# rpng/open_vins

Measured on AMD Instinct MI355X. Metric: MSCKF features/sec per EKF update (30-clone state), higher is better.
Workload: dtype f64; 1 GPU; BASELINE.json configs[2]: 2-camera radtan rig, 30-clone window, 2000 MSCKF features/update, N=248, D=208, online cam extrinsic+intrinsic calib + IMU intrinsics in the state, FEJ; features_total=2000, features_this_rank=2000, clones=30, cameras=2, state_dim=248, measurements_total=100362, parallelism=single GPU

## Files before the change

open_vins_amd/csrc/api_context.inc:

```
using namespace ovg;

static thread_local std::string g_err = "";
static int set_err(int code, const std::string &msg) {
  g_err = msg;
  return code;
}

#define HIPCHK(expr)                                                                                         \
  do {                                                                                                       \
    hipError_t _e = (expr);                                                                                  \
    if (_e != hipSuccess) {                                                                                  \
      return set_err(OVGPU_ERR_HIP, std::string(#expr) + " -> " + hipGetErrorString(_e) + " (" __FILE__ ":" + \
                                        std::to_string(__LINE__) + ")");                                     \
    }                                                                                                        \
  } while (0)

namespace {

template <class T>
struct PinBuf {
  T *p = nullptr;
  size_t cap = 0;
  hipError_t reserve(size_t n) {
    if (n <= cap) return hipSuccess;
// ... 234 lines not shown
  int tree_G = 0;
  bool tree_pipelined = true;
  int compress_gram = 1;
  DevBuf<double> gram_part, gram_G, gram_rho, Yaug2, Lw;
  double prior_pivot_tol = 1e-13;
  int last_route = OVGPU_COMPRESS_GRAM;
  bool whiten = true;
  bool gram_is_whitened = false;
  bool prior_on_side = false;
  int feat_variant = 0;
  int feat_nt_max = 0;
  bool featy_ok = false;
  int featy_skip = 0;
  int featy_grid = 0;
  size_t featy_lds = 0;
  DevBuf<double> fs_tq;
  DevBuf<int32_t> fs_inst;
  DevBuf<double> featyb_ws;
  int featy_big = 0;
  bool no_feat_kernel = false;
  bool raw_enable = true;
  bool gram_read_ahead = true;
  bool featy_chains = true;
  int raw_work_const = 12;
  bool raw_veto = false;
  bool raw_one_region = false;
  bool raw_cols_ok = false;
  bool raw_tables_ok = false;
  int raw_j0 = 0;
  int raw_ncls = 0, raw_ntc[RAW_MAXCLS + 1] = {0}, raw_ld[RAW_MAXCLS + 1] = {0}, raw_rcol[RAW_MAXCLS + 1] = {0};
  int64_t raw_base[RAW_MAXCLS + 1] = {0}, raw_rows[RAW_MAXCLS + 1] = {0};
  std::vector<uint8_t> h_cls_of_clone;
  DevBuf<uint8_t> cls_of_clone;
  DevBuf<int32_t> raw_featbase, raw_dst, raw_runs;
  DevBuf<double> Hraw;
  DevBuf<gram::GramRegionWG> gram_wg;
  int gram_wg_n = 0, gram_wg_tiles = 0;
  gram::GramRegionSum raw_rs;
  bool last_stack_raw = false;
  DevView<int32_t> feat_counter;
  DevBuf<int32_t> fs_minfo, fs_meas_feat, fs_pos;
  DevBuf<int32_t> fs_slots;
  std::vector<int32_t> h_order;
  std::vector<uint16_t> h_cc;
  DevBuf<double> fs_rows, fs_V, fs_z, fs_w;
  void *comm = nullptr;
// ... 344 lines not shown
```

open_vins_amd/csrc/api_debug.inc:

```
int ovgpu_debug_option(ovgpu_ctx *c, const char *name, int64_t value, int64_t *old_value) {
  if (!c || !name) return set_err(OVGPU_ERR_INVALID, "null argument");
  const std::string n(name);
  if (n == "chol_follow_spin_limit") {
    if (old_value) *old_value = c->chol_spin_limit;
    if (value >= 0) c->chol_spin_limit = (int)std::min<int64_t>(value, 1 << 30);
  } else if (n == "slam_chunked_fail_chunk") {
    if (old_value) *old_value = c->chunk_fail_inject;
    c->chunk_fail_inject = value >= 0 ? (int)std::min<int64_t>(value, 1 << 20) : -1;
  } else if (n == "slam_chunked_fallbacks") {
    if (old_value) *old_value = c->chunk_fallbacks;
    if (value >= 0) c->chunk_fallbacks = value;
  } else if (n == "delayed_init_fused") {
    if (old_value) *old_value = c->init_fused_on ? 1 : 0;
    if (value >= 0) c->init_fused_on = value != 0;
  } else if (n == "delayed_init_fused_steps") {
    if (old_value) *old_value = c->init_fused_steps;
    if (value >= 0) c->init_fused_steps = value;
  } else if (n == "delayed_init_chain_steps") {
    if (old_value) *old_value = c->init_chain_steps;
    if (value >= 0) c->init_chain_steps = value;
  } else if (n == "gram_interleaved") {
    if (old_value) *old_value = c->gram_il ? 1 : 0;
    if (value >= 0) c->gram_il = value != 0;
  } else if (n == "layout_fpw") {
// ... 34 lines not shown
    if (value >= 0) c->featy_big = (int)value;
  } else if (n == "upload_kernel") {
    if (old_value) *old_value = c->up_kernel;
    if (value >= 0) c->up_kernel = value != 0;
  } else if (n == "layout_every_update") {
    if (old_value) *old_value = c->layout_every_update;
    if (value >= 0) c->layout_every_update = value != 0;
  } else if (n == "tri_waves") {
    if (old_value) *old_value = c->tri_waves;
    if (value >= 0 && value <= 16) c->tri_waves = (int)value;
  } else if (n == "featy_skip") {
#ifdef OVG_FEAT_ABLATE
    if (old_value) *old_value = c->featy_skip;
    if (value >= 0) c->featy_skip = (int)value;
#else
    return set_err(OVGPU_ERR_INVALID, "featy_skip: ablation switches exist in a developer build only (-DOVG_FEAT_ABLATE)");
#endif
  } else if (n == "gram_read_ahead") {
    if (old_value) *old_value = c->gram_read_ahead ? 1 : 0;
    if (value >= 0) c->gram_read_ahead = value != 0;
  } else if (n == "featy_chains") {
    if (old_value) *old_value = c->featy_chains ? 1 : 0;
    if (value >= 0) c->featy_chains = value != 0;
  } else if (n == "raw_work_const") {
    if (old_value) *old_value = c->raw_work_const;
    if (value >= 0) c->raw_work_const = (int)value;
  } else if (n == "last_stack_raw") {
    if (old_value) *old_value = c->last_stack_raw ? 1 : 0;
  } else if (n == "raw_gram_tile_rows") {
    int64_t t = 0;
    if (c->raw_tables_ok)
      for (int k = 0; k <= RAW_NEG; k++) t += c->raw_rows[k] * (int64_t)(c->raw_ntc[k] * (c->raw_ntc[k] + 1) / 2);
    if (old_value) *old_value = t;
  } else if (n == "stack_is_f32") {
    if (old_value) *old_value = c->stack_is_f32 ? 1 : 0;
  } else if (n == "last_feature_kernel") {
    if (old_value) *old_value = c->last_feat_kernel;
  } else if (n == "last_gram_kernel") {
    if (old_value) *old_value = c->last_gram_kernel;
  } else if (n == "last_factor_kernel") {
    if (old_value) *old_value = c->last_factor_kernel;
  } else if (n == "last_unwhiten_kernel") {
    if (old_value) *old_value = c->last_unwhiten_kernel;
  } else if (n == "chol_wide") {
    if (old_value) *old_value = c->chol_wide ? 1 : 0;
    if (value >= 0) c->chol_wide = value != 0;
// ... 8 lines not shown
    if (old_value) *old_value = c->tsqr_last_leaf;
  } else if (n == "tsqr_last_tree") {
    if (old_value) *old_value = c->tsqr_last_tree;
  } else if (n == "tsqr_last_qh") {
    if (old_value) *old_value = c->tsqr_last_qh;
  } else if (n == "sys_lds_limit") {
    if (old_value) *old_value = c->lds_limit;
  } else if (n == "sys_m_lds_max") {
    if (old_value) *old_value = c->m_lds_max;
  } else if (n == "sys_rows_global") {
    if (old_value) *old_value = c->sys_rows_global ? 1 : 0;
  } else if (n == "sys_row_stride") {
    if (old_value) *old_value = c->row_stride;
  } else if (n == "sys_lds_bytes") {
    if (old_value) *old_value = (int64_t)c->sys_lds_bytes;
  } else if (n == "chol_timeouts") {
    if (old_value) *old_value = c->chol_timeouts;
  } else {
    return set_err(OVGPU_ERR_INVALID, "unknown debug option");
  }
  return OVGPU_OK;
}

int ovgpu_debug_cycles(ovgpu_ctx *c, int enable, long long *out512) {
  if (!c) return set_err(OVGPU_ERR_INVALID, "null ctx");
  HIPCHK(hipSetDevice(c->device));
  HIPCHK(upload_sync(c, c->stream));
  if (out512 && c->dbg_cycles.p) HIPCHK(hipMemcpy(out512, c->dbg_cycles.p, 512 * sizeof(long long), hipMemcpyDeviceToHost));
  if (enable) {
    HIPCHK(c->dbg_cycles.reserve(512));
    HIPCHK(hipMemset(c->dbg_cycles.p, 0, 512 * sizeof(long long)));
  } else if (!out512) {
    c->dbg_cycles.release();
  }
  return OVGPU_OK;
}

#ifdef OVG_GRAM_PROF
extern "C" int ovgpu_debug_gram_phases(ovgpu_ctx *c, long long *out, int workgroups, int *launched) {
  if (!c || !out || !launched || workgroups < 0 || workgroups > 1024) return set_err(OVGPU_ERR_INVALID, "bad argument");
  *launched = c->gram_wg_n;
  HIPCHK(hipSetDevice(c->device));
  HIPCHK(upload_sync(c, c->stream));
  HIPCHK(hipMemcpyFromSymbol(out, HIP_SYMBOL(gram::gram_prof_buf), sizeof(long long) * 32 * workgroups));
  return OVGPU_OK;
}
#endif

__global__ void k_clock_probe(long long *out, int iters) {
  const long long c0 = clock64(), w0 = wall_clock64();
  unsigned x = threadIdx.x + 1;
  for (int i = 0; i < iters; i++) x = x * 1664525u + 1013904223u;
  const long long c1 = clock64(), w1 = wall_clock64();
  if (threadIdx.x == 0) out[0] = c1 - c0, out[1] = w1 - w0, out[2] = (long long)x;
}
__global__ void __launch_bounds__(256) k_clock_probe_load(long long *out, int iters) {
  typedef double d4 __attribute__((ext_vector_type(4)));
  d4 a0 = {0, 0, 0, 0}, a1 = a0, a2 = a0, a3 = a0;
  const double x = 1.0 + 1e-9 * threadIdx.x, y = 1.0 - 1e-9 * threadIdx.x;
// ... 133 lines not shown
```

open_vins_amd/csrc/api_pipeline.inc:

```
static int enqueue_triangulate(ovgpu_ctx *c, const double *seed_pA = nullptr, const int32_t *seed_anchor = nullptr) {
  const Batch b = batch_of(c);
  if (b.F == 0) return OVGPU_OK;
  TriParams p;
  p.seed_pA = seed_pA, p.seed_anchor = seed_anchor, p.anchor_pre = c->anchor_pre.p;
  p.F = b.F, p.C = c->C, p.K = c->K;
  p.meas_offsets = b.meas_offsets, p.meas_cc = b.meas_cc, p.uvn = b.uvn, p.tab_cc = c->tab_cc.p;
  p.p_FinA = b.pA, p.p_FinG = b.pG, p.anchor_meas = c->anchor.p, p.status = b.status;
  p.opt = c->dopt;
  const size_t lds = (size_t)c->K * c->C * 12 * sizeof(double);
  int wpb = c->tri_waves;
  if (wpb == 0) {
    wpb = 4;
    const int room = c->num_cu - 6;
    for (int w = 4; w <= 8 && room > 0; w *= 2) {
      const int blocks = (b.F + w - 1) / w;
      if (blocks <= room) {
        if (4 * blocks >= 3 * room) wpb = w;
        break;
      }
    }
  }
  hipLaunchKernelGGL(k_triangulate, dim3((b.F + wpb - 1) / wpb), dim3(64 * wpb), lds, c->stream, p);
  HIPCHK(hipGetLastError());
  return OVGPU_OK;
}

extern "C++" {
template <int NW, int TPW, int OCC, bool F32, int CB, bool CH = false>
static int launch_featy(ovgpu_ctx *c, const SysParams &p, const double *sr, const int32_t *sm, const double *sV, const double *stq, const int32_t *sin, const int32_t *ssl) {
  static bool attr = false;
  auto kern = feat::k_feat_y<NW, TPW, OCC, F32, CB, CH>;
  if (!attr) {
    (void)hipFuncSetAttribute((const void *)kern, hipFuncAttributeMaxDynamicSharedMemorySize, c->lds_limit);
    attr = true;
  }
  const int nt = c->feat_nt_max, nta = c->feat_nta_max;
  if (nta * (nta + 1) / 2 > NW * TPW) return set_err(OVGPU_ERR_INVALID, "internal: the fused kernel's shape does not hold this batch's longest track");
  const size_t lds = feat::featy_lds_layout(nt, nta, NW, CB).total;
  if (lds > (size_t)c->lds_limit) return set_err(OVGPU_ERR_CAPACITY, "k_feat_y: track too long for its LDS block");
  const int per_cu = std::max(1, std::min(std::max(1, 4 * OCC / NW), (int)((size_t)c->lds_limit / lds)));
  const int grid = std::max(1, std::min(batch_of(c).F, c->num_cu * per_cu));
  hipLaunchKernelGGL(kern, dim3(grid), dim3(64 * NW), lds, c->stream, p, nt, nta, sr, sm, sV, stq, sin, ssl, (const int32_t *)c->raw_runs.p);
  return OVGPU_OK;
}
}

static int enqueue_system(ovgpu_ctx *c, int f_one = -1, int init_rep = 0, bool whiten = false) {
  const Batch b = batch_of(c);
  if (b.F == 0) return OVGPU_OK;
  SysParams p;
  p.F = b.F, p.C = c->C, p.K = c->K, p.D = c->D, p.LD = c->LD, p.N = c->N;
  p.meas_offsets = b.meas_offsets, p.meas_cc = b.meas_cc, p.uv = b.uv;
  p.tab_clone = c->tab_clone.p, p.tab_cam = c->tab_cam.p, p.intr = c->intr.p, p.fisheye = c->fisheye.p;
  p.clone_col = c->clone_col.p, p.calib_col = c->calib_col.p, p.intr_col = c->intr_col.p;
  p.col_cov = c->col_cov.p, p.col_kind = c->col_kind.p, p.col_var = c->col_var.p, p.col_sub = c->col_sub.p;
  p.P = c->P.p, p.p_FinG = b.pG, p.p_FinA = b.pA, p.anchor_meas = c->anchor.p;
  p.status = b.status, p.chi2 = b.chi2, p.chi2_thresh = b.chi2_thr;
  p.chi2_table = c->chi2_table.p, p.chi2_table_len = c->chi2_table_len;
  p.row_off = b.row_off, p.Hbig = c->Hbig.p, p.ws = c->gate_ws.p, p.ws_stride = c->gate_ws_stride;
  p.Hbig32 = nullptr, p.LDF = 0;
  c->stack_is_f32 = false;
  p.m_lds_max = c->m_lds_max, p.m_max = std::max(b.m_max, 1), p.row_stride = c->row_stride;
  p.opt = c->dopt;
  p.dbg = c->dbg_cycles.p ? c->dbg_cycles.p : qr_dbg_buffer();
// ... 51 lines not shown
        p.raw.on = 1, p.raw.ncls = c->raw_ncls, p.raw.H = c->Hraw.p, p.raw.dst = c->raw_dst.p, p.raw.j0 = c->raw_j0;
        for (int k = 0; k <= RAW_NEG; k++) p.raw.base[k] = c->raw_base[k], p.raw.ld[k] = c->raw_ld[k], p.raw.rcol[k] = c->raw_rcol[k];
        c->last_stack_raw = true;
      }
      if (c->inst_cb != cb || c->inst_D != c->D) {
        const int rci = enqueue_instance_lists(c, cb);
        if (rci != OVGPU_OK) return rci;
      }
      hipLaunchKernelGGL(feat::k_feat_vt, dim3((b.F + 3) / 4), dim3(256), (size_t)4 * (14 * p.m_max + 64) * sizeof(double), c->stream, p, st, c->fs_tq.p);
      if (c->prior_on_side) {
        HIPCHK(hipStreamWaitEvent(c->stream, c->ev_join, 0));
        c->prior_on_side = false;
      }
      const double *stq = c->fs_tq.p;
      const int32_t *sin = c->fs_inst.p, *ssl = c->fs_slots.p;
      if (big) {
        static bool attr_b = false;
        if (!attr_b) {
          (void)hipFuncSetAttribute((const void *)feat::k_feat_y_big<8, 17>, hipFuncAttributeMaxDynamicSharedMemorySize, c->lds_limit);
          (void)hipFuncSetAttribute((const void *)feat::k_feat_y_big<8, 17, true>, hipFuncAttributeMaxDynamicSharedMemorySize, c->lds_limit);
          (void)hipFuncSetAttribute((const void *)feat::k_feat_y_big<8, 5>, hipFuncAttributeMaxDynamicSharedMemorySize, c->lds_limit);
          attr_b = true;
        }
        const int nt = c->feat_nt_max, gridb = std::max(1, std::min(b.F, c->num_cu));
        const size_t ldsb = feat::featyb_lds_layout(nt, 8).total;
        if (ldsb > (size_t)c->lds_limit || nt > 29) return set_err(OVGPU_ERR_CAPACITY, "k_feat_y_big: track too long for its LDS block");
        HIPCHK(c->featyb_ws.reserve((size_t)gridb * feat::featyb_ws_doubles(nt)));
        if (c->featy_big == 2) hipLaunchKernelGGL((feat::k_feat_y_big<8, 5>), dim3(gridb), dim3(512), ldsb, c->stream, p, nt, sr, sm, sV, stq, sin, ssl, c->featyb_ws.p);
        else if (p.Hbig32) hipLaunchKernelGGL((feat::k_feat_y_big<8, 17, true>), dim3(gridb), dim3(512), ldsb, c->stream, p, nt, sr, sm, sV, stq, sin, ssl, c->featyb_ws.p);
        else hipLaunchKernelGGL((feat::k_feat_y_big<8, 17>), dim3(gridb), dim3(512), ldsb, c->stream, p, nt, sr, sm, sV, stq, sin, ssl, c->featyb_ws.p);
      } else {
        int rcl;
        if (c->feat_variant == 1 && p.Hbig32) rcl = launch_featy<4, 9, 2, true, 64>(c, p, sr, sm, sV, stq, sin, ssl);
        else if (c->feat_variant == 1) rcl = c->featy_chains ? launch_featy<4, 9, 2, false, 64, true>(c, p, sr, sm, sV, stq, sin, ssl) : launch_featy<4, 9, 2, false, 64>(c, p, sr, sm, sV, stq, sin, ssl);
        else if (p.Hbig32) rcl = launch_featy<8, 17, 1, true, 64>(c, p, sr, sm, sV, stq, sin, ssl);
        else rcl = c->featy_chains ? launch_featy<8, 17, 1, false, 64, true>(c, p, sr, sm, sV, stq, sin, ssl) : launch_featy<8, 17, 1, false, 64>(c, p, sr, sm, sV, stq, sin, ssl);
        if (rcl != OVGPU_OK) return rcl;
      }
      HIPCHK(hipGetLastError());
      return OVGPU_OK;
    }
    return set_err(OVGPU_ERR_INVALID, "internal: the MSCKF fast path was selected for a batch the fused kernel does not hold");
  }
  if (p.Lw && c->prior_on_side) {
    HIPCHK(hipStreamWaitEvent(c->stream, c->ev_join, 0));
    c->prior_on_side = false;
  }
// ... 982 lines not shown
```

open_vins_amd/csrc/api_state.inc:

```

const char *ovgpu_last_error(void) { return g_err.c_str(); }

void ovgpu_default_options(ovgpu_options *o) {
  if (!o) return;
  std::memset(o, 0, sizeof(*o));
  o->chi2_multipler = 5.0, o->sigma_pix = 1.0;
  o->triangulate_1d = 0, o->refine_features = 1, o->max_runs = 5;
  o->init_lamda = 1e-3, o->max_lamda = 1e10, o->min_dx = 1e-6, o->min_dcost = 1e-6, o->lam_mult = 10;
  o->min_dist = 0.10, o->max_dist = 60, o->max_baseline = 40, o->max_cond_number = 10000;
  o->do_fej = 1, o->do_calib_camera_pose = 1, o->do_calib_camera_intrinsics = 1;
  o->feat_rep_msckf = OVGPU_REP_GLOBAL_3D;
}

double ovgpu_chi2_quantile_95(int dof) { return chi2_quantile_95(dof); }
int ovgpu_abi_version(void) { return OVGPU_ABI_VERSION; }

int ovgpu_create(const ovgpu_options *opts, int device, ovgpu_ctx **out) {
  if (!opts || !out) return set_err(OVGPU_ERR_INVALID, "null argument");
  *out = nullptr;
  int ndev = 0;
  hipError_t e = hipGetDeviceCount(&ndev);
  if (e != hipSuccess || ndev <= 0)
    return set_err(OVGPU_ERR_NO_DEVICE, std::string("no HIP device (") + hipGetErrorString(e) + "): this library has no CPU fallback");
  if (device < 0 || device >= ndev) return set_err(OVGPU_ERR_INVALID, "device index out of range");
// ... 475 lines not shown
  c->inst_cb = lists ? cb : 0, c->inst_D = c->D;
  return OVGPU_OK;
}
static int enqueue_instance_lists(ovgpu_ctx *c, int cb) { return enqueue_batch_layout(c, false, cb); }
static int enqueue_batch_tables(ovgpu_ctx *c, bool anchors) { return enqueue_batch_layout(c, anchors, c->featy_ok ? featy_block_cols(c, featy_stack_f32(c, -1)) : feat::FY_CB); }

static int feature_rows(bool slam_rows, int m, int proj) { return slam_rows ? std::max(2 * m - proj, 0) : (m >= 2 ? 2 * m - 3 : 0); }
static void row_offsets_of(const ovgpu_ctx *c, const Batch &b, bool slam_rows, int64_t *out) {
  const int udof = lm_uniform_dof(c);
  out[0] = 0;
  for (int f = 0; f < b.F; f++) {
    int proj = udof == 1 ? 2 : 0;
    if (udof == 0 && (int)b.h_feat_lm.size() == b.F) proj = 3 - lm_dof(c->h_lm_rep[b.h_feat_lm[f]]);
    out[f + 1] = out[f] + feature_rows(slam_rows, b.h_offsets[f + 1] - b.h_offsets[f], proj);
  }
}
static void track_order(const int32_t *offsets, int F, int m_max, int32_t *order) {
  std::vector<int32_t> start(m_max + 2, 0);
  for (int f = 0; f < F; f++) start[m_max - (offsets[f + 1] - offsets[f]) + 1]++;
  for (int b = 0; b <= m_max; b++) start[b + 1] += start[b];
  for (int f = 0; f < F; f++) order[start[m_max - (offsets[f + 1] - offsets[f])]++] = f;
}

static int size_feature_stage(ovgpu_ctx *c) {
  const Batch b = batch_of(c);
  const int F = b.F, m_max = b.m_max;
  const bool slam_rows = c->slam_rows;
  size_t fixed = sys_lds_fixed_bytes(std::max(m_max, 1), c->row_stride, c->D);
  c->sys_rows_global = false;
  if (fixed >= (size_t)c->lds_limit) {
    fixed = sys_lds_fixed_bytes(std::max(m_max, 1), c->row_stride, c->D, false);
    c->sys_rows_global = true;
  }
  int m_lds = 0;
  if (fixed < (size_t)c->lds_limit) {
    const size_t avail = (size_t)c->lds_limit - fixed;
    while (m_lds < m_max && sys_gate_doubles(m_lds + 1) * sizeof(double) <= avail) m_lds++;
  } else {
    return set_err(OVGPU_ERR_CAPACITY, "track too long for the per-feature kernel's LDS tables (block ids and reflectors of ~1900 observations at 208 columns)");
  }
  c->m_lds_max = m_lds;
  c->sys_lds_bytes = fixed + sys_gate_doubles(m_lds) * sizeof(double);
  c->sys_grid = std::max(1, std::min(F, c->num_cu * 4));
  if (c->sys_rows_global) HIPCHK(c->sys_rows_ws.reserve((size_t)c->sys_grid * std::max(m_max, 1) * c->row_stride));
  if (m_lds < m_max) {
    c->gate_ws_stride = (int64_t)sys_gate_doubles(m_max);
// ... 3 lines not shown
  }
  c->feat_variant = 0;
  if (!slam_rows && !c->no_feat_kernel && (c->dopt.feat_rep < OVGPU_REP_ANCHORED_3D || c->anchored_fast) && (c->L == 0 || c->lm_empty_set) && m_max >= 2 && c->K * c->C <= 8192 && c->D >= 16) {
    const int nt = (2 * m_max + 15) / 16, nta = (2 * m_max + 4 + 15) / 16, tiles = nta * (nta + 1) / 2;
    int variant = tiles <= 4 * 9 ? 1 : (tiles <= 8 * 17 ? 2 : 0);
    if (c->feat_shape == 1 && tiles <= 4 * 9) variant = 1;
    if (c->feat_shape == 2 && tiles <= 8 * 17) variant = 2;
    c->feat_nta_max = nta;
    if (variant) {
      c->feat_variant = variant, c->feat_nt_max = nt;
    } else if (nt <= 29 && c->feat_shape == 0 && feat::featyb_lds_layout(nt, 8).total <= (size_t)c->lds_limit) {
      c->feat_variant = 3, c->feat_nt_max = nt;
    }
  }
  c->featy_ok = false;
  if (c->feat_variant) {
    const int nt = c->feat_nt_max, nw = c->feat_variant == 1 ? 4 : 8;
    const feat::FeatYLds lo = feat::featy_lds_layout(nt, c->feat_nta_max, nw, feat::FY_CB);
    const size_t vt_lds = (size_t)4 * (14 * std::max(m_max, 1) + 64) * sizeof(double);
    if (c->feat_variant == 3) {
      if (vt_lds <= (size_t)c->lds_limit) {
        c->featy_ok = true, c->featy_lds = feat::featyb_lds_layout(nt, 8).total;
        c->featy_grid = std::max(1, std::min(F, c->num_cu));
        HIPCHK(c->featyb_ws.reserve((size_t)c->featy_grid * feat::featyb_ws_doubles(nt)));
      } else {
        c->feat_variant = 0;
      }
    } else if (lo.total <= (size_t)c->lds_limit && vt_lds <= (size_t)c->lds_limit && c->feat_nta_max * (c->feat_nta_max + 1) / 2 <= nw * (nw == 4 ? 9 : 17)) {
      const int per_cu = nw == 4 ? std::max(1, std::min(2, (int)((size_t)c->lds_limit / lo.total))) : 1;
      c->featy_ok = true, c->featy_lds = lo.total;
      c->featy_grid = std::max(1, std::min(F, c->num_cu * per_cu));
    } else {
      c->feat_variant = 0;
    }
  }
  c->lm_fast_ok = c->L > 0 && c->feat_variant != 0 && c->featy_ok;
  c->slam_fused_ok = false, c->slam_fused_proj = false, c->slam_fused_long = false, c->slamy_lds = 0;
  const int slamy_mmax = c->slam_fused >= 3 ? slamy::SLY_MMAX_L : slamy::SLY_MMAX;
  if (slam_rows && c->slam_fused && !c->no_feat_kernel && c->L > 0 && m_max <= slamy_mmax && c->D >= 16 && c->K * c->C <= 8192) {
    const int udof = lm_uniform_dof(c);
    bool dof3 = udof == 3, named = udof != 0;
    if (udof == 0 && (int)b.h_feat_lm.size() == F) {
      dof3 = true, named = true;
      for (int f = 0; f < F; f++) dof3 = dof3 && lm_dof(c->h_lm_rep[b.h_feat_lm[f]]) == 3;
    }
    const bool proj = named && !dof3 && c->slam_fused >= 2;
    const bool lng = m_max > slamy::SLY_MMAX;
    const size_t lds = slamy::slamy_lds_layout(std::max(m_max, 1), proj, lng ? slamy::SLY_CB_L : slamy::SLY_CB).total;
    if ((dof3 || proj) && lds <= (size_t)c->lds_limit) c->slam_fused_ok = true, c->slam_fused_proj = proj, c->slam_fused_long = lng, c->slamy_lds = lds;
  }
  if (c->feat_variant) {
    const int M = std::max(b.M, 1);
    HIPCHK(c->fs_tq.reserve((size_t)std::max(F, 1) * 8));
    HIPCHK(c->fs_inst.reserve((size_t)std::max(F, 1) * std::max(c->feat_nt_max, 1) * feat::FY_ISTR));
    HIPCHK(c->fs_rows.reserve((size_t)M * c->row_stride));
    HIPCHK(c->fs_minfo.reserve((size_t)M * 8));
    HIPCHK(c->fs_V.reserve((size_t)M * 6));
    HIPCHK(c->fs_meas_feat.reserve(M));
    HIPCHK(c->fs_pos.reserve(M));
    std::vector<int32_t> slots((size_t)8 * std::max(F, 1), 0);
    for (int sidx = 0; sidx < F; sidx++) {
      const int f = b.h_order[sidx];
      const HostSpan<int64_t> &row_off = b.h_row_off;
      int32_t *r = &slots[(size_t)8 * sidx];
      r[0] = f, r[1] = b.h_offsets[f], r[2] = b.h_offsets[f + 1] - b.h_offsets[f], r[3] = (int32_t)(row_off[f + 1] - row_off[f]);
      r[4] = (int32_t)(uint32_t)((uint64_t)row_off[f] & 0xffffffffu), r[5] = (int32_t)(uint32_t)((uint64_t)row_off[f] >> 32);
    }
    HIPCHK(c->fs_slots.reserve(slots.size()));
    HIPCHK(upload_deferred(c, c->fs_slots.p, slots.data(), sizeof(int32_t) * slots.size()));
  }
  return configure_tsqr(c);
}

static int set_row_layout(ovgpu_ctx *c, bool slam_rows, bool anchors = false) {
  if (c->view) return set_err(OVGPU_ERR_INVALID, "internal: the resident batch cannot be laid out while a part of it is in force");
  const int F = c->F;
  c->h_row_off.resize(F + 1);
  row_offsets_of(c, batch_of(c), slam_rows, c->h_row_off.data());
  c->rows_total = c->h_row_off[F];
  c->slam_rows = slam_rows;
  const int rcs = size_feature_stage(c);
  if (rcs != OVGPU_OK) return rcs;
  HIPCHK(c->row_off.reserve(F + 1));
  HIPCHK(upload_deferred(c, c->row_off.p, c->h_row_off.data(), sizeof(int64_t) * (F + 1)));
  HIPCHK(upload_fence(c, c->stream));
  return enqueue_batch_tables(c, anchors);
}

static int raw_stack_layout(ovgpu_ctx *c, const uint16_t *cc) {
// ... 175 lines not shown
```

open_vins_amd/csrc/k_featy.h:

```cpp
#pragma once
#include <type_traits>

#include "k_feat.h"

namespace ovg {
namespace feat {

#ifdef OVG_FEAT_ABLATE
#define FY_SKIP(p) ((p).skip)
#else
#define FY_SKIP(p) 0
#endif
#ifndef FY_SYRK_UNROLL
#define FY_SYRK_UNROLL 2
#endif
constexpr int FY_CB = 64;
constexpr int FY_LS = 66;

struct FeatYLds {
  size_t yb, vl, wpart, misc, raw, total;
};
__host__ __device__ inline FeatYLds featy_lds_layout(int nt_max, int nta_max, int nw, int cb) {
  FeatYLds L;
  size_t o = 0;
// ... 29 lines not shown
  else dl[0] = 1, dl[1] = 0, dl[2] = 0, dl[3] = 0, dl[4] = 1, dl[5] = 0, dl[6] = 0, dl[7] = 0, dl[8] = 1;
  sys_measurement_rows(p, gm, p_FinG, p_FinG, false, hq, st.minfo + (size_t)8 * pos, st.rows + (size_t)pos * p.row_stride);
}

__global__ void __launch_bounds__(256) k_feat_rows_anchored(SysParams p, FeatStore st, int M) {
  const int gm = blockIdx.x * 256 + threadIdx.x;
  if (gm >= M) return;
  const int f = st.meas_feat[gm];
  if (p.status[f] != OVGPU_FEAT_USED) return;
  const int pos = st.pos[gm];
  const int ac = p.meas_cc[p.anchor_meas[f]];
  const double *tca = p.tab_cam + 12 * (ac >> 10), *tcl = p.tab_clone + 24 * (ac & 1023);
  const V3 p_FinA = load_v3(p.p_FinA + 3 * f);
  const V3 p_FinG = mulT(load_m3(tcl), mulT(load_m3(tca), p_FinA - load_v3(tca + 9))) + load_v3(tcl + 9);
  double hq[21], Ha[18], Hc[18];
  anchored_rep_jacobian(p.opt.feat_rep, p.opt.do_fej, tca, tcl, p_FinA, hq + 12, Ha, Hc);
  sys_measurement_rows(p, gm, p_FinG, p_FinG, false, hq, st.minfo + (size_t)8 * pos, st.rows + (size_t)pos * p.row_stride);
}
#endif

constexpr int FY_INST = 24;
constexpr int FY_ISTR = 32;
constexpr int FY_IOFF = 8;
constexpr int FY_RUNREC = RAW_MAXCLS + 1;
template <bool F32OUT>
__device__ __forceinline__ void vt_residual_column(const SysParams &p, int64_t orow0, const double *V, const double *res, int n, int lane, double z0, double z1,
                                                    double z2, double &sumsq, bool store = true) {
  const StackRows<F32OUT> out(p, orow0);
  double sq = 0.0;
  for (int r = 3 + lane; r < n; r += 64) {
    const double rp = res[r] - (V[3 * r] * z0 + V[3 * r + 1] * z1 + V[3 * r + 2] * z2);
    if (store) out.put(r - 3, p.D, rp);
    sq = fma(rp, rp, sq);
  }
  sumsq = wave_sum(sq);
}
__device__ __forceinline__ int64_t uniform_i64(int64_t v) {
  const uint32_t lo = __builtin_amdgcn_readfirstlane((uint32_t)(uint64_t)v), hi = __builtin_amdgcn_readfirstlane((uint32_t)((uint64_t)v >> 32));
  return (int64_t)(((uint64_t)hi << 32) | lo);
}
__device__ __forceinline__ void raw_region_of(const RawStack &rw, int d, int64_t &off, int &ld, int &rcol) {
  const int k = d >> RAW_CLS_SHIFT;
  int64_t base = rw.base[0];
  ld = rw.ld[0], rcol = rw.rcol[0];
#pragma unroll
  for (int q = 1; q < RAW_MAXCLS; q++)
// ... 385 lines not shown
  }
  int *rowlim = reinterpret_cast<int *>(smem + lo.misc + 32 * sizeof(double));
  int *sched = rowlim + nt_max;
  const double sig2 = p.opt.sigma_pix_sq;
  const int nblk = (D + CB - 1) / CB;

#ifdef OVG_FEAT_PROF
  long long tlast = 0;
  const bool prof = p.dbg != nullptr && blockIdx.x == 0 && tid == 0;
  if (prof) tlast = clock64();
#define FEAT_T(i)                              \
  if (prof) {                                  \
    const long long tn = clock64();            \
    p.dbg[220 + (i)] += tn - tlast, tlast = tn; \
  }
#define FEAT_TW(i)                                                  \
  if (prof) asm volatile("s_waitcnt vmcnt(0) lgkmcnt(0)" ::: "memory"); \
  FEAT_T(i)
#else
#define FEAT_T(i)
#define FEAT_TW(i)
#endif

  int nrec[6] = {0, 0, 0, 0, 0, 0}, nstatus = 0;
  if (CH && (int)blockIdx.x < p.F) {
    const int32_t *rec = slotsG + (size_t)8 * blockIdx.x;
#pragma unroll
    for (int q = 0; q < 6; q++) nrec[q] = rec[q];
    if (CHX) nstatus = p.status[nrec[0]];
  }
  for (int slot = blockIdx.x; slot < p.F; slot += gridDim.x) {
    lds_barrier();
    const int32_t *rec = slotsG + (size_t)8 * slot;
    const int f = __builtin_amdgcn_readfirstlane(CH ? nrec[0] : rec[0]);
    const int m0 = __builtin_amdgcn_readfirstlane(CH ? nrec[1] : rec[1]);
    const int m = __builtin_amdgcn_readfirstlane(CH ? nrec[2] : rec[2]);
    const int n_out = __builtin_amdgcn_readfirstlane(CH ? nrec[3] : rec[3]);
    const int64_t orow0 = (int64_t)(((uint64_t)(uint32_t)__builtin_amdgcn_readfirstlane(CH ? nrec[5] : rec[5]) << 32) | (uint32_t)__builtin_amdgcn_readfirstlane(CH ? nrec[4] : rec[4]));
    const StackRows<F32OUT> out(p, orow0);
    const int n = 2 * m;
    int status_f = 0;
    i32x4 rr = {0, 0, 0, 0};
    double T00, T01, T02, T11, T12, T22, bound, thr;
    auto head_loads = [&]() {
      const double *tq = tqG + (size_t)8 * f;
      T00 = tq[0], T01 = tq[1], T02 = tq[2], T11 = tq[3], T12 = tq[4], T22 = tq[5];
      bound = tq[6];
      thr = p.opt.chi2_multipler * p.chi2_table[min(max(n - 3, 0), p.chi2_table_len - 1)];
      const int nchunk = (24 * n + 1023) >> 10;
      const char *src = reinterpret_cast<const char *>(VG + (size_t)6 * m0);
      for (int ch = wv; ch < nchunk; ch += NW) {
        const int off = min(1024 * ch + 16 * lane, 24 * n - 16);
        __builtin_amdgcn_global_load_lds((const __attribute__((address_space(1))) void *)(src + off),
                                         (__attribute__((address_space(3))) void *)(reinterpret_cast<char *>(Vl) + 1024 * ch), 16, 0, 0);
      }
    };
    const bool has_next = slot + (int)gridDim.x < p.F;
    if (CH) {
      status_f = CHX ? nstatus : p.status[f];
      if (raw && CHX) rr = reinterpret_cast<const i32x4 *>(runsG)[(size_t)f * FY_RUNREC + min(lane, RAW_MAXCLS)];
      head_loads();
    }
    if (CH && has_next) {
      const int32_t *nx = slotsG + (size_t)8 * (slot + gridDim.x);
#pragma unroll
      for (int q = 0; q < 6; q++) nrec[q] = nx[q];
    }
    if (raw && !CH) {
      if (tid < RAW_MAXCLS) clsbeg[tid] = -1;
      lds_barrier();
      if (tid < m) {
        const int d = p.raw.dst[m0 + tid], k = d >> RAW_CLS_SHIFT, kp = tid > 0 ? (p.raw.dst[m0 + tid - 1] >> RAW_CLS_SHIFT) : -1;
        if (k != kp) clsbeg[k] = tid, clsbeg[k + 8] = d & RAW_ROW_MASK;
      }
      lds_barrier();
      if (tid == 0) {
        int hi = m, nr = 0;
#pragma unroll
        for (int k = RAW_MAXCLS - 1; k >= 0; k--) {
          const int lo_m = clsbeg[k];
          if (lo_m >= 0) {
            const int ls = rawld[k];
            const int64_t off = rawbase[k] + (int64_t)clsbeg[k + 8] * (ls & 0xffff);
            runs[nr++] = i32x4{(2 * lo_m) | ((2 * hi) << 16), ls, (int)(uint32_t)(uint64_t)off, (int)(uint32_t)((uint64_t)off >> 32)};
            hi = lo_m;
          }
        }
        *nruns = nr;
      }
// ... 249 lines not shown
          if (g + 4 * q == cl) acc[s][q] += sig2;
      }
    }
    FEAT_T(4)
    const double chi2 = skip_gate ? bound : ((FY_SKIP(p) & 8) ? 0.0 : gate_ldl_chi2<NW, TPW>(acc, tij, NT, NTA, n, panel, panelx, st0, stE, stF, chi2_slot, lane, wv));
    if (wv == 0 && lane == 0) {
      if (skip_gate && p.rows_used) atomicAdd(p.rows_used + 1, 1);
      p.chi2[f] = chi2;
      p.chi2_thresh[f] = thr;
      const bool reject = chi2 > thr;
      sched[1] = reject ? 1 : 0;
      if (reject) p.status[f] = OVGPU_FEAT_CHI2_REJECTED;
      else if (p.rows_used) atomicAdd(p.rows_used, n_out);
    }
    lds_barrier();
    if (sched[1]) {
      __syncthreads();
      if (raw) raw_zero();
      else
        for (int64_t e = tid; e < (int64_t)n_out * out.ld; e += NTH) out.zero(e);
    }
    FEAT_T(5)
  }
#undef FEAT_T
#undef FEAT_TW
#undef TI
#undef TJ
}

#define OVG_FEATY_SHAPES(X)                                                                                                     \
  X(4, 9, 2, false, 64, false) X(4, 9, 2, true, 64, false) X(8, 17, 1, false, 64, false) X(8, 17, 1, true, 64, false) \
  X(4, 9, 2, false, 64, true) X(8, 17, 1, false, 64, true)
#define OVG_FEATY_ARGS                                                                                                                           \
  SysParams, int, int, const double *__restrict__, const int32_t *__restrict__, const double *__restrict__, const double *__restrict__, \
      const int32_t *__restrict__, const int32_t *__restrict__, const int32_t *__restrict__

}
}
```

open_vins_amd/csrc/k_featy_big.h:

```cpp
#pragma once
#include "k_featy.h"

namespace ovg {
namespace feat {

constexpr int FB_CB = 32;
constexpr int FB_LS = 34;
constexpr int FB_PF = 15;

struct FeatYBigLds {
  size_t yb, vl, wpart, rhs, misc, total;
};
__host__ __device__ inline FeatYBigLds featyb_lds_layout(int nt_max, int nw) {
  FeatYBigLds L;
  size_t o = 0;
  auto take = [&](size_t bytes) {
    const size_t at = o;
    o += (bytes + 15) & ~(size_t)15;
    return at;
  };
  const size_t blk = (size_t)16 * nt_max * FB_LS * sizeof(double), pan = (size_t)2 * (nt_max + 1) * 256 * sizeof(double);
  L.yb = take(blk > pan ? blk : pan);
  L.vl = take((((size_t)16 * nt_max * 3 * sizeof(double)) + 1023) & ~(size_t)1023);
  const size_t wp = (size_t)nw * 3 * FB_CB * sizeof(double), stage = 2 * 256 * sizeof(double);
// ... 12 lines not shown
  extern __shared__ __attribute__((aligned(16))) unsigned char smem[];
  constexpr int NTH = 64 * NW;
  static_assert(FB_PF * NTH >= 30 * 256, "a fetched row panel must fit the prefetch registers");
  const int tid = threadIdx.x, lane = tid & 63;
  const int wv = __builtin_amdgcn_readfirstlane(tid >> 6);
  const int g = lane >> 4, cl = lane & 15;
  const int D = p.D, LD = p.LD, RS = p.row_stride;
  const FeatYBigLds lo = featyb_lds_layout(nt_max, NW);
  double *Yb = reinterpret_cast<double *>(smem + lo.yb);
  double *panel0 = Yb, *panel1 = Yb + (size_t)(nt_max + 1) * 256;
  double *Vl = reinterpret_cast<double *>(smem + lo.vl);
  double *wpart = reinterpret_cast<double *>(smem + lo.wpart);
  double *st0 = wpart, *st1 = wpart + 256;
  double *rhs = reinterpret_cast<double *>(smem + lo.rhs);
  double *zres = reinterpret_cast<double *>(smem + lo.misc);
  int *rowlim = reinterpret_cast<int *>(smem + lo.misc + 32 * sizeof(double));
  int *sched = rowlim + nt_max;
  double *ws = wsG + (size_t)blockIdx.x * featyb_ws_doubles(nt_max);
  const double sig2 = p.opt.sigma_pix_sq;
  const int nblk = (D + FB_CB - 1) / FB_CB;
  const int col32 = lane & 31, hp = lane >> 5;
  auto ld_l2 = [](const double *ptr) { return __hip_atomic_load(ptr, __ATOMIC_RELAXED, __HIP_MEMORY_SCOPE_AGENT); };

  for (int slot = blockIdx.x; slot < p.F; slot += gridDim.x) {
    lds_barrier();
    const int32_t *rec = slotsG + (size_t)8 * slot;
    const int f = __builtin_amdgcn_readfirstlane(rec[0]);
    const int m0 = __builtin_amdgcn_readfirstlane(rec[1]);
    const int m = __builtin_amdgcn_readfirstlane(rec[2]);
    const int n_out = __builtin_amdgcn_readfirstlane(rec[3]);
    const int64_t orow0 = (int64_t)(((uint64_t)(uint32_t)__builtin_amdgcn_readfirstlane(rec[5]) << 32) | (uint32_t)__builtin_amdgcn_readfirstlane(rec[4]));
    const StackRows<F32OUT> out(p, orow0);
    if (p.status[f] != OVGPU_FEAT_USED) {
      for (int64_t e = tid; e < (int64_t)n_out * out.ld; e += NTH) out.zero(e);
      continue;
    }
    const int n = 2 * m, NT = (n + 15) >> 4;
    const double *frow = rowsG + (size_t)m0 * RS;
    const int32_t *finfo = minfoG + (size_t)8 * m0;
    const double *fV = VG + (size_t)6 * m0;
    const double T00 = tqG[(size_t)8 * f], T01 = tqG[(size_t)8 * f + 1], T02 = tqG[(size_t)8 * f + 2], T11 = tqG[(size_t)8 * f + 3],
                 T12 = tqG[(size_t)8 * f + 4], T22 = tqG[(size_t)8 * f + 5];

    {
      const int nchunk = (24 * n + 1023) >> 10;
      const char *src = reinterpret_cast<const char *>(fV);
      for (int ch = wv; ch < nchunk; ch += NW) {
        const int off = min(1024 * ch + 16 * lane, 24 * n - 16);
        __builtin_amdgcn_global_load_lds((const __attribute__((address_space(1))) void *)(src + off),
                                         (__attribute__((address_space(3))) void *)(reinterpret_cast<char *>(Vl) + 1024 * ch), 16, 0, 0);
// ... 280 lines not shown
        g0 = fma(y0, yr, g0), g1 = fma(y1, yr, g1), g2 = fma(y2, yr, g2);
      }
      sa = wave_sum(sa);
      G00 = wave_sum(G00), G01 = wave_sum(G01), G02 = wave_sum(G02), G11 = wave_sum(G11), G12 = wave_sum(G12), G22 = wave_sum(G22);
      g0 = wave_sum(g0), g1 = wave_sum(g1), g2 = wave_sum(g2);
      const M3 Gm{G00, G01, G02, G01, G11, G12, G02, G12, G22};
      const V3 gv{g0, g1, g2};
      const V3 x = colpiv_qr_solve3(Gm, gv);
      const double chi2 = sa - dot(gv, x);
      if (lane == 0) {
        p.chi2[f] = chi2;
        p.chi2_thresh[f] = thr;
        const bool reject = chi2 > thr;
        sched[1] = reject ? 1 : 0;
        if (reject) p.status[f] = OVGPU_FEAT_CHI2_REJECTED;
        else if (p.rows_used) atomicAdd(p.rows_used, n_out);
      }
    }
    lds_barrier();
    if (sched[1]) {
      for (int64_t e = tid; e < (int64_t)n_out * out.ld; e += NTH) out.zero(e);
    }
  }
}

}
}
```

Before: 2.944 million features/s.

## Deal feature slots to workgroups by modeled cost via linked slot lists

Replaces the fixed grid-stride slot loop in the feature kernels with per-workgroup linked lists stored in each slot record, built on the host. With the new featy_deal option, slots are assigned from a per-track-length cost model by a row-wise dealer with rebalancing, falling back to LPT when imbalance is high. The aim is to shrink the tail where one workgroup holds the longest tracks. By default featy_deal is off, so the lists reproduce round-robin and only the traversal mechanism changes. Also adds optional per-slot cycle profiling and a grid-cap knob.

```diff
diff --git a/open_vins_amd/csrc/api_context.inc b/open_vins_amd/csrc/api_context.inc
--- a/open_vins_amd/csrc/api_context.inc
+++ b/open_vins_amd/csrc/api_context.inc
@@ -280,6 +280,10 @@
   bool raw_enable = true;
   bool gram_read_ahead = true;
   bool featy_chains = true;
+  bool featy_deal = false;
+  int featy_grid_cap = 0;
+  int64_t featy_deal_permille = 0;
+  std::vector<int32_t> deal_cost, deal_link, deal_lut;
   int raw_work_const = 12;
   bool raw_veto = false;
   bool raw_one_region = false;
diff --git a/open_vins_amd/csrc/api_debug.inc b/open_vins_amd/csrc/api_debug.inc
--- a/open_vins_amd/csrc/api_debug.inc
+++ b/open_vins_amd/csrc/api_debug.inc
@@ -80,6 +80,14 @@
   } else if (n == "featy_chains") {
     if (old_value) *old_value = c->featy_chains ? 1 : 0;
     if (value >= 0) c->featy_chains = value != 0;
+  } else if (n == "featy_deal") {
+    if (old_value) *old_value = c->featy_deal ? 1 : 0;
+    if (value >= 0) c->featy_deal = value != 0;
+  } else if (n == "featy_grid_cap") {
+    if (old_value) *old_value = c->featy_grid_cap;
+    if (value >= 0) c->featy_grid_cap = (int)std::min<int64_t>(value, 1 << 20);
+  } else if (n == "featy_deal_imbalance_permille") {
+    if (old_value) *old_value = c->featy_deal_permille;
   } else if (n == "raw_work_const") {
     if (old_value) *old_value = c->raw_work_const;
     if (value >= 0) c->raw_work_const = (int)value;
@@ -134,19 +142,35 @@
   return OVGPU_OK;
 }
 
+#ifdef OVG_FEAT_PROF
+constexpr size_t DBG_CYCLES_LEN = 512 + feat::FY_PROF_SLOTS;
+#else
+constexpr size_t DBG_CYCLES_LEN = 512;
+#endif
 int ovgpu_debug_cycles(ovgpu_ctx *c, int enable, long long *out512) {
   if (!c) return set_err(OVGPU_ERR_INVALID, "null ctx");
   HIPCHK(hipSetDevice(c->device));
   HIPCHK(upload_sync(c, c->stream));
   if (out512 && c->dbg_cycles.p) HIPCHK(hipMemcpy(out512, c->dbg_cycles.p, 512 * sizeof(long long), hipMemcpyDeviceToHost));
   if (enable) {
-    HIPCHK(c->dbg_cycles.reserve(512));
-    HIPCHK(hipMemset(c->dbg_cycles.p, 0, 512 * sizeof(long long)));
+    HIPCHK(c->dbg_cycles.reserve(DBG_CYCLES_LEN));
+    HIPCHK(hipMemset(c->dbg_cycles.p, 0, DBG_CYCLES_LEN * sizeof(long long)));
   } else if (!out512) {
     c->dbg_cycles.release();
   }
   return OVGPU_OK;
 }
+
+#ifdef OVG_FEAT_PROF
+extern "C" int ovgpu_debug_slot_cycles(ovgpu_ctx *c, long long *out, int32_t *slots8, int n) {
+  if (!c || !out || n < 0 || n > feat::FY_PROF_SLOTS || !c->dbg_cycles.p) return set_err(OVGPU_ERR_INVALID, "bad argument, or the counters are not enabled");
+  HIPCHK(hipSetDevice(c->device));
+  HIPCHK(upload_sync(c, c->stream));
+  HIPCHK(hipMemcpy(out, c->dbg_cycles.p + 512, n * sizeof(long long), hipMemcpyDeviceToHost));
+  if (slots8 && c->fs_slots.p) HIPCHK(hipMemcpy(slots8, c->fs_slots.p, (size_t)n * 8 * sizeof(int32_t), hipMemcpyDeviceToHost));
+  return OVGPU_OK;
+}
+#endif
 
 #ifdef OVG_GRAM_PROF
 extern "C" int ovgpu_debug_gram_phases(ovgpu_ctx *c, long long *out, int workgroups, int *launched) {
diff --git a/open_vins_amd/csrc/api_pipeline.inc b/open_vins_amd/csrc/api_pipeline.inc
--- a/open_vins_amd/csrc/api_pipeline.inc
+++ b/open_vins_amd/csrc/api_pipeline.inc
@@ -39,7 +39,8 @@
   const size_t lds = feat::featy_lds_layout(nt, nta, NW, CB).total;
   if (lds > (size_t)c->lds_limit) return set_err(OVGPU_ERR_CAPACITY, "k_feat_y: track too long for its LDS block");
   const int per_cu = std::max(1, std::min(std::max(1, 4 * OCC / NW), (int)((size_t)c->lds_limit / lds)));
-  const int grid = std::max(1, std::min(batch_of(c).F, c->num_cu * per_cu));
+  const int grid = c->featy_grid;
+  if (grid < 1 || grid > std::max(1, std::min(batch_of(c).F, c->num_cu * per_cu))) return set_err(OVGPU_ERR_INVALID, "internal: the slot lists were dealt for another grid than this shape's");
   hipLaunchKernelGGL(kern, dim3(grid), dim3(64 * NW), lds, c->stream, p, nt, nta, sr, sm, sV, stq, sin, ssl, (const int32_t *)c->raw_runs.p);
   return OVGPU_OK;
 }
@@ -137,7 +138,8 @@
           (void)hipFuncSetAttribute((const void *)feat::k_feat_y_big<8, 5>, hipFuncAttributeMaxDynamicSharedMemorySize, c->lds_limit);
           attr_b = true;
         }
-        const int nt = c->feat_nt_max, gridb = std::max(1, std::min(b.F, c->num_cu));
+        const int nt = c->feat_nt_max, gridb = c->featy_grid;
+        if (gridb < 1 || gridb > b.F) return set_err(OVGPU_ERR_INVALID, "internal: the slot lists were dealt for another batch");
         const size_t ldsb = feat::featyb_lds_layout(nt, 8).total;
         if (ldsb > (size_t)c->lds_limit || nt > 29) return set_err(OVGPU_ERR_CAPACITY, "k_feat_y_big: track too long for its LDS block");
         HIPCHK(c->featyb_ws.reserve((size_t)gridb * feat::featyb_ws_doubles(nt)));
diff --git a/open_vins_amd/csrc/api_state.inc b/open_vins_amd/csrc/api_state.inc
--- a/open_vins_amd/csrc/api_state.inc
+++ b/open_vins_amd/csrc/api_state.inc
@@ -521,6 +521,10 @@
   for (int f = 0; f < F; f++) order[start[m_max - (offsets[f + 1] - offsets[f])]++] = f;
 }
 
+extern "C++" {
+#include "slot_deal.h"
+}
+
 static int size_feature_stage(ovgpu_ctx *c) {
   const Batch b = batch_of(c);
   const int F = b.F, m_max = b.m_max;
@@ -570,6 +574,7 @@
       if (vt_lds <= (size_t)c->lds_limit) {
         c->featy_ok = true, c->featy_lds = feat::featyb_lds_layout(nt, 8).total;
         c->featy_grid = std::max(1, std::min(F, c->num_cu));
+        if (c->featy_grid_cap > 0) c->featy_grid = std::min(c->featy_grid, c->featy_grid_cap);
         HIPCHK(c->featyb_ws.reserve((size_t)c->featy_grid * feat::featyb_ws_doubles(nt)));
       } else {
         c->feat_variant = 0;
@@ -578,6 +583,7 @@
       const int per_cu = nw == 4 ? std::max(1, std::min(2, (int)((size_t)c->lds_limit / lo.total))) : 1;
       c->featy_ok = true, c->featy_lds = lo.total;
       c->featy_grid = std::max(1, std::min(F, c->num_cu * per_cu));
+      if (c->featy_grid_cap > 0) c->featy_grid = std::min(c->featy_grid, c->featy_grid_cap);
     } else {
       c->feat_variant = 0;
     }
@@ -606,13 +612,30 @@
     HIPCHK(c->fs_V.reserve((size_t)M * 6));
     HIPCHK(c->fs_meas_feat.reserve(M));
     HIPCHK(c->fs_pos.reserve(M));
+    const int G = std::max(1, c->featy_grid);
+    c->deal_link.resize(std::max(F, 1)), c->deal_cost.resize(std::max(F, 1));
+    deal::cost_table(c->feat_variant == 1 ? deal::COST_FEATY_4_9_2 : (c->feat_variant == 2 ? deal::COST_FEATY_8_17_1 : deal::COST_FEATY_BIG), std::max(m_max, 0), c->deal_lut);
     std::vector<int32_t> slots((size_t)8 * std::max(F, 1), 0);
+    bool by_cost = c->featy_deal;
     for (int sidx = 0; sidx < F; sidx++) {
       const int f = b.h_order[sidx];
       const HostSpan<int64_t> &row_off = b.h_row_off;
       int32_t *r = &slots[(size_t)8 * sidx];
       r[0] = f, r[1] = b.h_offsets[f], r[2] = b.h_offsets[f + 1] - b.h_offsets[f], r[3] = (int32_t)(row_off[f + 1] - row_off[f]);
       r[4] = (int32_t)(uint32_t)((uint64_t)row_off[f] & 0xffffffffu), r[5] = (int32_t)(uint32_t)((uint64_t)row_off[f] >> 32);
+      c->deal_cost[sidx] = c->deal_lut[std::min(std::max(r[2], 0), std::max(m_max, 0))];
+      by_cost = by_cost && (sidx == 0 || c->deal_cost[sidx] <= c->deal_cost[sidx - 1]);
+    }
+    c->featy_deal_permille = 0;
+    if (F > 0) {
+      static thread_local deal::DealScratch scratch;
+      if (by_cost) {
+        c->featy_deal_permille = deal::deal_by_cost(c->deal_cost.data(), F, G, c->deal_link.data(), scratch).permille();
+      } else {
+        deal::deal_round_robin(F, G, c->deal_link.data());
+        c->featy_deal_permille = deal::measure_lists(c->deal_cost.data(), F, G, c->deal_link.data()).permille();
+      }
+      for (int sidx = 0; sidx < F; sidx++) slots[(size_t)8 * sidx + 6] = c->deal_link[sidx];
     }
     HIPCHK(c->fs_slots.reserve(slots.size()));
     HIPCHK(upload_deferred(c, c->fs_slots.p, slots.data(), sizeof(int32_t) * slots.size()));
diff --git a/open_vins_amd/csrc/k_featy.h b/open_vins_amd/csrc/k_featy.h
--- a/open_vins_amd/csrc/k_featy.h
+++ b/open_vins_amd/csrc/k_featy.h
@@ -75,6 +75,7 @@
 constexpr int FY_INST = 24;
 constexpr int FY_ISTR = 32;
 constexpr int FY_IOFF = 8;
+constexpr int FY_PROF_SLOTS = 16384;
 constexpr int FY_RUNREC = RAW_MAXCLS + 1;
 template <bool F32OUT>
 __device__ __forceinline__ void vt_residual_column(const SysParams &p, int64_t orow0, const double *V, const double *res, int n, int lane, double z0, double z1,
@@ -506,16 +507,31 @@
 #define FEAT_TW(i)
 #endif
 
-  int nrec[6] = {0, 0, 0, 0, 0, 0}, nstatus = 0;
+  int nrec[7] = {0, 0, 0, 0, 0, 0, -1}, nstatus = 0;
   if (CH && (int)blockIdx.x < p.F) {
     const int32_t *rec = slotsG + (size_t)8 * blockIdx.x;
 #pragma unroll
-    for (int q = 0; q < 6; q++) nrec[q] = rec[q];
+    for (int q = 0; q < 7; q++) nrec[q] = rec[q];
     if (CHX) nstatus = p.status[nrec[0]];
   }
-  for (int slot = blockIdx.x; slot < p.F; slot += gridDim.x) {
+#ifdef OVG_FEAT_PROF
+  const bool profs = p.dbg != nullptr && tid == 0;
+  long long ts_slot = 0;
+  int f_slot = -1;
+#define FEAT_SLOT_T(fnext)                                                                     \
+  if (profs) {                                                                                 \
+    const long long tn = clock64();                                                            \
+    if (f_slot >= 0 && f_slot < FY_PROF_SLOTS) p.dbg[512 + f_slot] += tn - ts_slot;             \
+    ts_slot = tn, f_slot = (fnext);                                                            \
+  }
+#else
+#define FEAT_SLOT_T(fnext)
+#endif
+  int next = -1;
+  for (int slot = (int)blockIdx.x < p.F ? (int)blockIdx.x : -1; slot >= 0; slot = next) {
     lds_barrier();
     const int32_t *rec = slotsG + (size_t)8 * slot;
+    next = __builtin_amdgcn_readfirstlane(CH ? nrec[6] : rec[6]);
     const int f = __builtin_amdgcn_readfirstlane(CH ? nrec[0] : rec[0]);
     const int m0 = __builtin_amdgcn_readfirstlane(CH ? nrec[1] : rec[1]);
     const int m = __builtin_amdgcn_readfirstlane(CH ? nrec[2] : rec[2]);
@@ -539,16 +555,17 @@
                                          (__attribute__((address_space(3))) void *)(reinterpret_cast<char *>(Vl) + 1024 * ch), 16, 0, 0);
       }
     };
-    const bool has_next = slot + (int)gridDim.x < p.F;
+    const bool has_next = next >= 0;
+    FEAT_SLOT_T(f)
     if (CH) {
       status_f = CHX ? nstatus : p.status[f];
       if (raw && CHX) rr = reinterpret_cast<const i32x4 *>(runsG)[(size_t)f * FY_RUNREC + min(lane, RAW_MAXCLS)];
       head_loads();
     }
     if (CH && has_next) {
-      const int32_t *nx = slotsG + (size_t)8 * (slot + gridDim.x);
-#pragma unroll
-      for (int q = 0; q < 6; q++) nrec[q] = nx[q];
+      const int32_t *nx = slotsG + (size_t)8 * next;
+#pragma unroll
+      for (int q = 0; q < 7; q++) nrec[q] = nx[q];
     }
     if (raw && !CH) {
       if (tid < RAW_MAXCLS) clsbeg[tid] = -1;
@@ -844,6 +861,8 @@
     }
     FEAT_T(5)
   }
+  FEAT_SLOT_T(-1)
+#undef FEAT_SLOT_T
 #undef FEAT_T
 #undef FEAT_TW
 #undef TI
diff --git a/open_vins_amd/csrc/k_featy_big.h b/open_vins_amd/csrc/k_featy_big.h
--- a/open_vins_amd/csrc/k_featy_big.h
+++ b/open_vins_amd/csrc/k_featy_big.h
@@ -58,10 +58,26 @@
   const int col32 = lane & 31, hp = lane >> 5;
   auto ld_l2 = [](const double *ptr) { return __hip_atomic_load(ptr, __ATOMIC_RELAXED, __HIP_MEMORY_SCOPE_AGENT); };
 
-  for (int slot = blockIdx.x; slot < p.F; slot += gridDim.x) {
+#ifdef OVG_FEAT_PROF
+  const bool profs = p.dbg != nullptr && tid == 0;
+  long long ts_slot = 0;
+  int f_slot = -1;
+#define FEATB_SLOT_T(fnext)                                                        \
+  if (profs) {                                                                     \
+    const long long tn = clock64();                                                \
+    if (f_slot >= 0 && f_slot < FY_PROF_SLOTS) p.dbg[512 + f_slot] += tn - ts_slot; \
+    ts_slot = tn, f_slot = (fnext);                                                \
+  }
+#else
+#define FEATB_SLOT_T(fnext)
+#endif
+  int next = -1;
+  for (int slot = (int)blockIdx.x < p.F ? (int)blockIdx.x : -1; slot >= 0; slot = next) {
     lds_barrier();
     const int32_t *rec = slotsG + (size_t)8 * slot;
     const int f = __builtin_amdgcn_readfirstlane(rec[0]);
+    next = __builtin_amdgcn_readfirstlane(rec[6]);
+    FEATB_SLOT_T(f)
     const int m0 = __builtin_amdgcn_readfirstlane(rec[1]);
     const int m = __builtin_amdgcn_readfirstlane(rec[2]);
     const int n_out = __builtin_amdgcn_readfirstlane(rec[3]);
@@ -388,6 +404,8 @@
       for (int64_t e = tid; e < (int64_t)n_out * out.ld; e += NTH) out.zero(e);
     }
   }
+  FEATB_SLOT_T(-1)
+#undef FEATB_SLOT_T
 }
 
 }
diff --git a/open_vins_amd/csrc/slot_deal.h b/open_vins_amd/csrc/slot_deal.h
--- /dev/null
+++ b/open_vins_amd/csrc/slot_deal.h
@@ -0,0 +1,194 @@
+#pragma once
+#include <algorithm>
+#include <cstdint>
+#include <utility>
+#include <vector>
+
+namespace ovg {
+namespace deal {
+
+constexpr int DEAL_MAX_MOVES = 64;
+
+struct DealScratch {
+  std::vector<int64_t> load;
+  std::vector<int32_t> tail, perm, link2;
+};
+struct DealResult {
+  int lists = 0;
+  int64_t busiest = 0;
+  int64_t total = 0;
+  int moves = 0;
+  int64_t permille() const { return total > 0 ? (1000 * busiest * lists + total / 2) / total : 1000; }
+};
+
+inline bool costs_non_increasing(const int32_t *cost, int F) {
+  for (int i = 1; i < F; i++)
+    if (cost[i] > cost[i - 1]) return false;
+  return true;
+}
+
+inline DealResult measure_lists(const int32_t *cost, int F, int G, const int32_t *link) {
+  DealResult r;
+  r.lists = std::min(F, G);
+  for (int b = 0; b < r.lists; b++) {
+    int64_t s = 0;
+    for (int i = b; i >= 0; i = link[i]) s += cost[i];
+    r.busiest = std::max(r.busiest, s), r.total += s;
+  }
+  return r;
+}
+
+inline void deal_round_robin(int F, int G, int32_t *link) {
+  for (int i = 0; i < F; i++) link[i] = i + G < F ? i + G : -1;
+}
+
+inline DealResult deal_rows(const int32_t *cost, int F, int G, int32_t *link, DealScratch &s) {
+  DealResult res;
+  if (F <= 0 || G <= 0) return res;
+  const int L = std::min(F, G);
+  res.lists = L;
+  s.load.resize(L), s.tail.resize(L);
+  int64_t *load = s.load.data();
+  int32_t *tail = s.tail.data();
+  std::fill(link, link + F, -1);
+  for (int b = 0; b < L; b++) load[b] = cost[b];
+  bool counted = true, t_fwd = true;
+  int t_lo = 0;
+  auto write_tails = [&]() {
+    if (!counted) return;
+    if (t_fwd) for (int b = 0; b < L; b++) tail[b] = t_lo + b;
+    else for (int b = 0; b < L; b++) tail[b] = t_lo + G - 1 - b;
+    counted = false;
+  };
+  enum { FLAT, FALLING, RISING, NONE };
+  int state = cost[0] == cost[L - 1] ? FLAT : FALLING;
+  int64_t base = 0;
+  for (int lo = G; lo < F; lo += G) {
+    const int hi = std::min(F, lo + G), r = hi - lo;
+    const bool one_cost = cost[lo] == cost[hi - 1], same_to_all = one_cost && r == G;
+    const int32_t *cr = cost + lo;
+    if (state == NONE && !same_to_all) {
+      write_tails();
+      s.perm.resize(L);
+      int32_t *perm = s.perm.data();
+      for (int b = 0; b < L; b++) perm[b] = b;
+      std::stable_sort(perm, perm + L, [&](int32_t x, int32_t y) { return load[x] < load[y]; });
+      for (int j = 0; j < r; j++) {
+        const int b = perm[j];
+        link[tail[b]] = lo + j, tail[b] = lo + j, load[b] += cr[j];
+      }
+    } else {
+      const bool fwd = same_to_all || state != FALLING;
+      if (r == G && counted) {
+        int32_t *lk = link + t_lo;
+        if (fwd == t_fwd) for (int j = 0; j < G; j++) lk[j] = lo + j;
+        else for (int j = 0; j < G; j++) lk[G - 1 - j] = lo + j;
+        t_lo = lo, t_fwd = fwd;
+      } else {
+        write_tails();
+        if (fwd) for (int j = 0; j < r; j++) link[tail[j]] = lo + j, tail[j] = lo + j;
+        else for (int j = 0; j < r; j++) link[tail[G - 1 - j]] = lo + j, tail[G - 1 - j] = lo + j;
+      }
+      if (same_to_all) {
+        base += cr[0];
+        continue;
+      }
+      if (fwd) for (int j = 0; j < r; j++) load[j] += cr[j];
+      else for (int j = 0; j < r; j++) load[G - 1 - j] += cr[j];
+    }
+    if (hi < F) {
+      if (state == FLAT) {
+        state = one_cost ? FLAT : FALLING;
+      } else {
+        bool falling = true, rising = true;
+        for (int b = 1; b < G; b++) falling = falling && load[b] <= load[b - 1], rising = rising && load[b] >= load[b - 1];
+        state = falling && rising ? FLAT : (falling ? FALLING : (rising ? RISING : NONE));
+      }
+    }
+  }
+  write_tails();
+  int a = 0, z = 0;
+  auto extremes = [&]() {
+    a = z = 0;
+    for (int b = 1; b < L; b++) {
+      if (load[b] > load[a]) a = b;
+      if (load[b] < load[z]) z = b;
+    }
+  };
+  extremes();
+  while (res.moves < DEAL_MAX_MOVES) {
+    const int t = tail[a];
+    if (t < G || load[z] + cost[t] >= load[a]) break;
+    int pa = a;
+    while (link[pa] != t) pa = link[pa];
+    link[pa] = -1, tail[a] = pa, load[a] -= cost[t];
+    int pz = z;
+    while (link[pz] >= 0 && link[pz] < t) pz = link[pz];
+    link[t] = link[pz], link[pz] = t, load[z] += cost[t];
+    if (link[t] < 0) tail[z] = t;
+    res.moves++;
+    extremes();
+  }
+  res.busiest = load[a] + base;
+  for (int b = 0; b < L; b++) res.total += load[b];
+  res.total += base * L;
+  return res;
+}
+
+inline DealResult deal_lpt(const int32_t *cost, int F, int G, int32_t *link, DealScratch &s) {
+  DealResult res;
+  if (F <= 0 || G <= 0) return res;
+  const int L = std::min(F, G);
+  res.lists = L;
+  s.tail.assign(L, -1);
+  typedef std::pair<int64_t, int32_t> Entry;
+  std::vector<Entry> heap;
+  heap.reserve(L);
+  for (int b = 0; b < L; b++) heap.emplace_back(0, b);
+  auto later = [](const Entry &x, const Entry &y) { return x > y; };
+  for (int i = 0; i < F; i++) {
+    std::pop_heap(heap.begin(), heap.end(), later);
+    Entry &e = heap.back();
+    if (s.tail[e.second] >= 0) link[s.tail[e.second]] = i;
+    link[i] = -1, s.tail[e.second] = i, e.first += cost[i];
+    res.total += cost[i];
+    std::push_heap(heap.begin(), heap.end(), later);
+  }
+  for (const Entry &e : heap) res.busiest = std::max(res.busiest, e.first);
+  return res;
+}
+
+constexpr int DEAL_LPT_PERCENT = 105;
+inline DealResult deal_by_cost(const int32_t *cost, int F, int G, int32_t *link, DealScratch &s) {
+  DealResult res = deal_rows(cost, F, G, link, s);
+  if (res.lists == 0) return res;
+  const int64_t bound = std::max<int64_t>(cost[0], (res.total + res.lists - 1) / res.lists);
+  if (res.busiest * 100 > bound * DEAL_LPT_PERCENT) {
+    s.link2.resize(F);
+    const DealResult lpt = deal_lpt(cost, F, G, s.link2.data(), s);
+    if (lpt.busiest < res.busiest) {
+      std::copy(s.link2.begin(), s.link2.end(), link);
+      res = lpt, res.moves = -1;
+    }
+  }
+  return res;
+}
+
+struct SlotCostModel {
+  int32_t c0, c1, c2;
+  int32_t rows[9];
+};
+constexpr SlotCostModel COST_FEATY_4_9_2{0, 1500, 0, {5000, 65250, 64250, 70250, 62250, 79250, 123250, 121250, 125000}};
+constexpr SlotCostModel COST_FEATY_8_17_1{35824, 2388, 8, {0, 0, 0, 0, 0, 0, 0, 0, 0}};
+constexpr SlotCostModel COST_FEATY_BIG{53273, 2945, 7, {0, 0, 0, 0, 0, 0, 0, 0, 0}};
+inline void cost_table(const SlotCostModel &k, int m_max, std::vector<int32_t> &lut) {
+  lut.resize((size_t)std::max(m_max, 0) + 1);
+  int64_t best = 0;
+  for (int m = 0; m <= m_max; m++) {
+    best = std::max<int64_t>(best, (int64_t)k.c0 + (int64_t)k.c1 * m + (int64_t)k.c2 * m * m + k.rows[std::min((m + 7) / 8, 8)]);
+    lut[m] = (int32_t)std::min<int64_t>(best, INT32_MAX / 4);
+  }
+}
+
+}
+}
```

New measurement: 2.934 million features/s. No clear change (-0.3%).
